# harryjfowen/PointsToWood

Measured on AMD Instinct MI355X. Metric: classified points/sec, higher is better.
Workload: dtype f16x3

## Files before the change

### pointstowood_amd/csrc/p2w_hgemm.h

```cpp
#pragma once
#include "p2w_common.h"
#include <type_traits>

typedef float f32x16 __attribute__((ext_vector_type(16)));
typedef _Float16 h8 __attribute__((ext_vector_type(8)));
typedef __bf16 bf8 __attribute__((ext_vector_type(8)));
typedef __fp16 hpair __attribute__((ext_vector_type(2)));
typedef _Float16 hpairn __attribute__((ext_vector_type(2)));
typedef __bf16 bpair __attribute__((ext_vector_type(2)));
typedef float fpair __attribute__((ext_vector_type(2)));
typedef __attribute__((address_space(3))) void* lds_vp;
typedef const __attribute__((address_space(1))) void* glb_vp;

constexpr int H_BK = 32;
constexpr int SA_EPI_COLS = 1024;

template <int PREC> struct HCfg {
    static constexpr int planes = PREC == 0 ? 2 : 1;
    static constexpr int kslab = PREC == 0 ? 32 : 64;
    static constexpr int kalign = PREC == 0 ? 32 : 64;
};

template <int PREC>
__device__ __forceinline__ f32x16 h_mfma(h8 a, h8 b, f32x16 c) {
    if constexpr (PREC == 2)
        return __builtin_amdgcn_mfma_f32_32x32x16_bf16(__builtin_bit_cast(bf8, a), __builtin_bit_cast(bf8, b), c, 0, 0, 0);
    else
        return __builtin_amdgcn_mfma_f32_32x32x16_f16(a, b, c, 0, 0, 0);
}

typedef float f32x4 __attribute__((ext_vector_type(4)));
template <int PREC>
__device__ __forceinline__ f32x4 h_mfma16(h8 a, h8 b, f32x4 c) {
    if constexpr (PREC == 2)
        return __builtin_amdgcn_mfma_f32_16x16x32_bf16(__builtin_bit_cast(bf8, a), __builtin_bit_cast(bf8, b), c, 0, 0, 0);
    else
        return __builtin_amdgcn_mfma_f32_16x16x32_f16(a, b, c, 0, 0, 0);
}

__device__ __forceinline__ void split_pair(float a, float b, unsigned& hi, unsigned& lo) {
    const hpair h = __builtin_amdgcn_cvt_pkrtz(a, b);
    const fpair rem = {a - (float)h[0], b - (float)h[1]};
    const hpairn l = __builtin_convertvector(rem, hpairn);
    hi = __builtin_bit_cast(unsigned, h);
    lo = __builtin_bit_cast(unsigned, l);
}
template <int PREC>
__device__ __forceinline__ unsigned pack_pair(float a, float b) {
    if constexpr (PREC == 2) {
        const fpair p = {a, b};
        return __builtin_bit_cast(unsigned, __builtin_convertvector(p, bpair));
    } else {
        const fpair p = {__builtin_amdgcn_fmed3f(a, -65504.f, 65504.f), __builtin_amdgcn_fmed3f(b, -65504.f, 65504.f)};
        return __builtin_bit_cast(unsigned, __builtin_convertvector(p, hpairn));
    }
}
template <int PREC>
__device__ __forceinline__ void h_store2(_Float16* __restrict__ base, unsigned ldh, unsigned row, unsigned col, float a, float b) {
    if constexpr (PREC == 0) {
        unsigned hw, lw;
        split_pair(a, b, hw, lw);
        _Float16* p = base + (size_t)row * (2 * ldh) + 64 * (col >> 5) + (col & 31);
        *reinterpret_cast<unsigned*>(p) = hw;
        *reinterpret_cast<unsigned*>(p + 32) = lw;
    } else {
        *reinterpret_cast<unsigned*>(base + (size_t)row * ldh + col) = pack_pair<PREC>(a, b);
    }
}
template <int PREC>
__device__ __forceinline__ void h_store4(_Float16* __restrict__ base, int ldh, size_t row, int col, const float (&v)[4]) {
    if constexpr (PREC == 0) {
        uint2 hi, lo;
        split_pair(v[0], v[1], hi.x, lo.x);
        split_pair(v[2], v[3], hi.y, lo.y);
        _Float16* p = base + row * (size_t)(2 * ldh) + 64 * (col >> 5) + (col & 31);
        *reinterpret_cast<uint2*>(p) = hi;
        *reinterpret_cast<uint2*>(p + 32) = lo;
    } else {
        uint2 w;
        w.x = pack_pair<PREC>(v[0], v[1]);
        w.y = pack_pair<PREC>(v[2], v[3]);
        *reinterpret_cast<uint2*>(base + row * (size_t)ldh + col) = w;
    }
}

__device__ __forceinline__ bool tile_coords_at(int L, int nMt, int nNt, int* mt, int* nt, int mode = 0) {
    const int xcd = L & 7, w = L >> 3;
    if (mode == 0) {
        *mt = xcd + 8 * (w / nNt);
        *nt = w % nNt;
        return *mt < nMt;
    }
    if (nNt >= 8) {
        const int cpx = (nNt + 7) >> 3;
        *mt = w / cpx;
        *nt = xcd + 8 * (w % cpx);
        return *mt < nMt && *nt < nNt;
    }
    const int r = 8 / nNt;
    *nt = xcd % nNt;
    *mt = xcd / nNt + r * w;
    return *mt < nMt;
}
__device__ __forceinline__ bool tile_coords(int nMt, int nNt, int* mt, int* nt, int mode = 0) {
    return tile_coords_at(blockIdx.x, nMt, nNt, mt, nt, mode);
}
static inline int tile_grid(int nMt, int nNt, int mode = 0) {
    if (mode == 0) return 8 * ((nMt + 7) / 8) * nNt;
    if (nNt >= 8) return 8 * nMt * ((nNt + 7) / 8);
    const int r = 8 / nNt;
    return 8 * ((nMt + r - 1) / r);
}
static inline int p2w_cu_count() {
    int dev = 0, n = 256;
    if (hipGetDevice(&dev) == hipSuccess) hipDeviceGetAttribute(&n, hipDeviceAttributeMultiprocessorCount, dev);
    return n > 0 ? n : 256;
}

constexpr int RI_DEPTH = 2;
struct EpiArgs {
    const float *bias, *sc0, *sh0, *sc1, *sh1, *residual;
    int ldr, relu0, relu1, relu2, relu_final;
    const _Float16* res_h;
    unsigned* range;
    const int4* imeta;
};
__device__ __forceinline__ void range_commit(unsigned* __restrict__ dst, bool over, bool seen, int lane) {
    if (lane == 0) {
        unsigned* p = dst + (blockIdx.x & (P2W_RANGE_SLOTS - 1)) * 64;
        if (over) p[0] = 1u;
        if (seen) p[1] = 1u;
    }
}
__device__ __forceinline__ void range_commit_max(unsigned* __restrict__ dst, float m, int lane) {
    range_commit(dst, __ballot(!(m <= P2W_RANGE_HI)) != 0ull, __ballot(m > P2W_RANGE_LO) != 0ull, lane);
}
template <int PREC>
__device__ __forceinline__ fpair h_load2(const _Float16* __restrict__ base, unsigned ldh, unsigned row, unsigned col) {
    if constexpr (PREC == 0) {
        const _Float16* p = base + (size_t)row * (2 * ldh) + 64 * (col >> 5) + (col & 31);
        const hpairn hi = *reinterpret_cast<const hpairn*>(p), lo = *reinterpret_cast<const hpairn*>(p + 32);
        return fpair{(float)hi[0] + (float)lo[0], (float)hi[1] + (float)lo[1]};
    } else if constexpr (PREC == 1) {
        const hpairn v = *reinterpret_cast<const hpairn*>(base + (size_t)row * ldh + col);
        return fpair{(float)v[0], (float)v[1]};
    } else {
        const bpair v = *reinterpret_cast<const bpair*>(base + (size_t)row * ldh + col);
        return fpair{(float)v[0], (float)v[1]};
    }
}
struct OutArgs { float* f32; int ldo; _Float16* h2; int ldh; int hcols; const float* dotw; float* part; int ldpart; };

__device__ __forceinline__ float row16_sum(float v) {
    asm volatile("s_nop 4\n\t"
                 "v_add_f32_dpp %0, %0, %0 quad_perm:[1,0,3,2] row_mask:0xf bank_mask:0xf bound_ctrl:1\n\ts_nop 1\n\t"
                 "v_add_f32_dpp %0, %0, %0 quad_perm:[2,3,0,1] row_mask:0xf bank_mask:0xf bound_ctrl:1\n\ts_nop 1\n\t"
                 "v_add_f32_dpp %0, %0, %0 row_half_mirror row_mask:0xf bank_mask:0xf bound_ctrl:1\n\ts_nop 1\n\t"
                 "v_add_f32_dpp %0, %0, %0 row_mirror row_mask:0xf bank_mask:0xf bound_ctrl:1\n\ts_nop 1"
                 : "+v"(v));
    return v;
}

__device__ __forceinline__ int w_stage_row16(int rho) {
    const int t = rho >> 4, c = rho & 15;
    return 32 * (t >> 1) + 2 * c + (t & 1);
}

template <int PREC, int RT16, int CT16, int EF, bool DOTK = false>
__device__ __forceinline__ void gemm_epilogue_16(const f32x4 (&acc)[RT16][CT16], const EpiArgs& ep, float wscale, int row0, int col0,
                                                 int lane, int M, int N, const OutArgs& o, bool seen_report = true) {
    static_assert(CT16 % 2 == 0, "column tiles come in interleaved pairs");
    constexpr bool GEN = EF < 0;
    constexpr int JQ = CT16 / 2, NSTEP = RT16 * 4;
    const bool R0 = GEN ? ep.relu0 != 0 : (EF & 1) != 0, S0 = GEN ? ep.sc0 != nullptr : (EF & 2) != 0;
    const bool R1 = GEN ? ep.relu1 != 0 : (EF & 4) != 0, S1 = GEN ? ep.sc1 != nullptr : (EF & 8) != 0;
    const bool R2 = GEN ? ep.relu2 != 0 : (EF & 16) != 0;
    const bool RES = !DOTK && (GEN ? (ep.residual != nullptr || ep.res_h != nullptr) : (EF & 32) != 0);
    const bool RF = GEN ? ep.relu_final != 0 : (EF & 64) != 0, OF = GEN ? o.f32 != nullptr : (EF & 128) != 0;
    const bool OH = GEN ? o.h2 != nullptr : (EF & 256) != 0;
    const bool RH = RES && (GEN ? ep.res_h != nullptr : (EF & 1024) != 0);
    constexpr bool RI_OK = !DOTK && RT16 <= 4;
    const bool RI = RI_OK && RES && (GEN ? ep.imeta != nullptr : (EF & 2048) != 0);
// ... 440 lines not shown
    if (out_h2 && (ldh_o & 7)) return P2W_EINVAL;
    const int hcols = ldh_o < (N + KA - 1) / KA * KA ? ldh_o : (N + KA - 1) / KA * KA;
    OutArgs o = {out_f32, ldo, out_h2, ldh_o, hcols, dotw, part, ldpart};
    const int n_cu = p2w_cu_count();
    auto pick_big = [&](int rows) {
        const long tiles256 = (long)p2w_cdiv(rows, 256) * (Npad / 256);
        const long rounds = (tiles256 + n_cu - 1) / n_cu;
        const bool fills = tiles256 * 100 >= rounds * n_cu * 78;
        bool b = N >= 256 && (N % 256) == 0 && tiles256 * 4 >= 3 * n_cu && fills;
        if (flags & P2W_GEMM_TILE_256) b = true;
        if (flags & P2W_GEMM_TILE_128) b = false;
        return b;
    };
    const bool big = pick_big(M);
    bool t64 = false;
    if (!dotw && sk_S == 0 && !ep.imeta && !(flags & (P2W_GEMM_TILE_128 | P2W_GEMM_TILE_256 | P2W_GEMM_NO_TILE_64))) {
        if (flags & P2W_GEMM_TILE_64) t64 = true;
        else if (K <= 1024 && N <= 192) t64 = true;
        else if (K <= 1024 && !big) {
            const long nNt1 = p2w_cdiv(N, 128), T128 = (long)p2w_cdiv(M, 128) * nNt1, T64 = (long)p2w_cdiv(M, 64) * nNt1;
            const long S128 = 2L * n_cu, S64 = 3L * n_cu;
            const double w128 = (double)((T128 + S128 - 1) / S128 * S128) / (double)T128, w64 = (double)((T64 + S64 - 1) / S64 * S64) / (double)T64;
            t64 = T128 <= 2 * S128 && w128 >= 1.3 * w64;
        }
    }
    if (sk_S == 0 && skws && !dotw && !t64 && !(flags & P2W_GEMM_NO_STREAMK)) {
        const int nslab = Kpad / HCfg<PREC>::kslab;
        const double f = PREC == 0 ? 1.0 : 0.7, ts1 = 0.9 * f, ts2 = 1.65 * f, tsb = 2.25 * f;
        auto t_small = [&](long tiles) { return tiles > n_cu ? ts2 : ts1; };
        auto t_big = [&](long tiles) { return tiles >= n_cu ? tsb : (0.75 * f + (tsb - 0.75 * f) * (double)tiles / n_cu); };
        auto one_launch = [&](bool b, int rows) {
            const long T = b ? (long)p2w_cdiv(rows, 256) * (Npad / 256) : (long)p2w_cdiv(rows, 128) * p2w_cdiv(N, 128);
            const long G = b ? n_cu : 2 * n_cu, qq = T / G, R = T % G;
            return (double)nslab * ((double)qq * (b ? tsb : ts2) + (R ? (b ? t_big(R) : t_small(R)) : 0.0));
        };
        const bool big_ok = N >= 256 && (N % 256) == 0;
        double best_cost = one_launch(big, M);
        int best_mode = 0, best_rows_full = 0, best_S = 0;
        bool best_big = big, sk_big = big, tail_big = false;
        double sk_cost = 1e30;
        int sk_rows_full = 0, sk_S_best = 0;
        const size_t piece_b = (size_t)128 * 128 * 4;
        for (int cand = 0; cand < 2; ++cand) {
            const bool b = cand == 0;
            if (b && !(N >= 256 && (N % 256) == 0)) continue;
            if ((flags & P2W_GEMM_TILE_256) && !b) continue;
            if ((flags & P2W_GEMM_TILE_128) && b) continue;
            const int BMm = b ? 256 : 128, G_m = n_cu * (b ? 1 : 2);
            const int nNt_m = b ? Npad / 256 : p2w_cdiv(N, 128), nMt_m = p2w_cdiv(M, BMm);
            const long T = (long)nMt_m * nNt_m, q = T / G_m;
            const int mt_full = (int)((q * G_m) / nNt_m);
            if ((long)mt_full * nNt_m >= T) continue;
            if (q == 0 && b != big) continue;
            const int rows_full = mt_full * BMm, m_t = M - rows_full;
            const double main_t = (double)q * nslab * (b ? tsb : ts2) + (q > 0 ? 4.0 : 0.0);
            const long T_t = (long)p2w_cdiv(m_t, 128) * p2w_cdiv(N, 128);
            if (q > 0) {
                for (int tb = 0; tb < 2; ++tb) {
                    if (tb == 1 && (!big_ok || (flags & P2W_GEMM_TILE_128))) continue;
                    if (tb == 0 && (flags & P2W_GEMM_TILE_256)) continue;
                    const double c = main_t + one_launch(tb == 1, m_t);
                    if (c < 0.95 * best_cost) { best_cost = c; best_mode = 1; best_rows_full = rows_full; best_big = b; best_S = 0; tail_big = tb == 1; }
                }
            }
            for (int S = 2; S <= nslab && T_t * S <= 2 * n_cu; ++S) {
                if ((size_t)(T_t * S) * piece_b > skws_bytes) break;
                const double c = main_t + (double)((nslab + S - 1) / S) * 1.0 * f + 18.0 + (double)(T_t * S) * piece_b * 2.0 / 8.0e6;
                if (c < sk_cost) { sk_cost = c; sk_rows_full = rows_full; sk_big = b; sk_S_best = S; }
            }
        }
        if (sk_S_best > 0 && (sk_cost < 0.9 * best_cost || (flags & P2W_GEMM_STREAMK))) {
            best_mode = 2; best_rows_full = sk_rows_full; best_big = sk_big; best_S = sk_S_best;
        }
        if (best_mode != 0) {
            constexpr int PL = HCfg<PREC>::planes;
            const int fl = (flags & ~(P2W_GEMM_STREAMK | P2W_GEMM_TILE_128 | P2W_GEMM_TILE_256)) | P2W_GEMM_NO_STREAMK;
            const int rows_full = best_rows_full, m_t = M - rows_full;
            if (rows_full > 0) {
                const int32_t rc = launch_gemm_h<PREC>(Ah, ldh_a, Wp, wscale, rows_full, N, K, ep, out_f32, ldo, out_h2, ldh_o,
                                                       fl | (best_big ? P2W_GEMM_TILE_256 : P2W_GEMM_TILE_128), stream);
                if (rc != P2W_OK) return rc;
            }
            const size_t r0 = (size_t)rows_full;
            EpiArgs ept = ep;
            if (ept.imeta) ept.imeta += r0;
            else if (ept.residual) ept.residual += r0 * ep.ldr;
            if (ept.res_h) ept.res_h += r0 * PL * ep.ldr;
            return launch_gemm_h<PREC>(Ah + r0 * PL * ldh_a, ldh_a, Wp, wscale, m_t, N, K, ept, out_f32 ? out_f32 + r0 * ldo : nullptr, ldo,
                                       out_h2 ? out_h2 + r0 * PL * ldh_o : nullptr, ldh_o,
                                       best_mode == 2 ? fl : (fl | (tail_big ? P2W_GEMM_TILE_256 : P2W_GEMM_TILE_128)), stream, nullptr, nullptr, 0,
                                       best_mode == 2 ? skws : nullptr, skws_bytes, best_mode == 2 ? best_S : 0);
        }
    }
    int ef = (ep.relu0 ? 1 : 0) | (ep.sc0 ? 2 : 0) | (ep.relu1 ? 4 : 0) | (ep.sc1 ? 8 : 0) | (ep.relu2 ? 16 : 0) |
             ((ep.residual || ep.res_h) ? 32 : 0) | (ep.relu_final ? 64 : 0) | (out_f32 ? 128 : 0) | (out_h2 ? 256 : 0) | (dotw ? 512 : 0) |
             (ep.res_h ? 1024 : 0) | (ep.imeta ? 2048 : 0);
    const size_t lim = (size_t)1 << 31;
    if ((size_t)M * (size_t)(ldo > 2 * ldh_o ? ldo : 2 * ldh_o) >= lim || ((ep.residual || ep.res_h) && !ep.imeta && (size_t)M * (size_t)ep.ldr * (ep.res_h ? 2 : 1) >= lim) ||
        (N & 1) || (flags & P2W_GEMM_GENERIC_EPI))
        ef = 0;
    auto odd8 = [](const void* q) { return (reinterpret_cast<uintptr_t>(q) & 7) != 0; };
    if ((out_f32 && ((ldo & 1) || odd8(out_f32))) || (ep.residual && ((ep.ldr & 1) || odd8(ep.residual))) || odd8(ep.bias) ||
        (ep.res_h && ((ep.ldr & 7) || (reinterpret_cast<uintptr_t>(ep.res_h) & 15))) ||
        odd8(ep.sc0) || odd8(ep.sh0) || odd8(ep.sc1) || odd8(ep.sh1) || odd8(dotw) || (part && ((ldpart & 3) || (reinterpret_cast<uintptr_t>(part) & 15))))
        ef = 0;
    const size_t w_bytes = (size_t)N * Kpad * 2 * HCfg<PREC>::planes, a_bytes = (size_t)M * Kpad * 2 * HCfg<PREC>::planes;
    auto pick_mode = [&](int nNtx, int nMtx, int per_cu) {
        const bool ok = nNtx >= 8 || (nNtx > 0 && 8 % nNtx == 0);
        if (!ok) return 0;
        if (flags & P2W_GEMM_ORDER_ROWS) return 0;
        if (flags & P2W_GEMM_ORDER_COLS) return 1;
        const size_t l2_keep = (size_t)3 * 1024 * 1024;
        const int wpx = n_cu / 8 * per_cu;
        const int R = wpx / nNtx > 0 ? wpx / nNtx : 1;
        const int rows_px = p2w_cdiv(nMtx, 8), xcds = nMtx < 8 ? nMtx : 8;
        const size_t t_rows = a_bytes * (size_t)p2w_cdiv(nNtx, wpx) + w_bytes * xcds * (w_bytes <= l2_keep ? 1 : p2w_cdiv(rows_px, R));
        size_t t_cols;
        if (nNtx >= 8) {
            const int cpx = p2w_cdiv(nNtx, 8), Rc = wpx / cpx > 0 ? wpx / cpx : 1;
            t_cols = a_bytes * 8 + w_bytes * (w_bytes / 8 <= l2_keep ? 1 : p2w_cdiv(nMtx, Rc));
        } else {
            t_cols = a_bytes * nNtx + w_bytes * 8 / nNtx;
        }
        return t_cols * 10 < t_rows * 9 ? 1 : 0;
    };
    auto pgrid = [&](int nvb, int per_cu) {
        const int cap = n_cu * per_cu;
        int g = nvb < cap ? nvb : cap;
        if (g >= 8) g &= ~7;
        return g;
    };
    if (sk_S > 0) {
        const int nslab = Kpad / HCfg<PREC>::kslab, nNt1 = p2w_cdiv(N, 128), T_t = p2w_cdiv(M, 128) * nNt1;
        gemm_hp_sk_kernel<PREC, 2, 2, 2, 2><<<8 * p2w_cdiv(T_t * sk_S, 8), 256, 0, stream>>>(Ah, ldh_a, Wp, M, Kpad, nNt1, T_t, sk_S, skws);
        gemm_hp_skfix_kernel<PREC, 2, 2, 2, 2><<<T_t * 4, 256, 0, stream>>>(skws, T_t, sk_S, nslab, nNt1, wscale, M, N, ep, o, ef);
    } else if (t64) {
        const int nMt = p2w_cdiv(M, 64), nNt1 = p2w_cdiv(N, 128);
        const int tm = pick_mode(nNt1, nMt, 3), nvb = tile_grid(nMt, nNt1, tm);
        gemm_hp64_kernel<PREC><<<pgrid(nvb, 3), 256, 0, stream>>>(Ah, ldh_a, Wp, wscale, M, N, Kpad, nMt, nNt1, nvb, ep, o, ef, tm);
    } else if (big) {
        const int nMt = p2w_cdiv(M, 256), nNt2 = Npad / 256;
        const int tm = pick_mode(nNt2, nMt, 1), nvb = tile_grid(nMt, nNt2, tm);
        if (dotw) gemm_hp_kernel<PREC, 2, 4, 4, 2, true><<<pgrid(nvb, 1), 512, 0, stream>>>(Ah, ldh_a, Wp, wscale, M, N, Kpad, nMt, nNt2, nvb, ep, o, ef, tm);
        else gemm_hp_kernel<PREC, 2, 4, 4, 2><<<pgrid(nvb, 1), 512, 0, stream>>>(Ah, ldh_a, Wp, wscale, M, N, Kpad, nMt, nNt2, nvb, ep, o, ef, tm);
    } else {
        const int nMt = p2w_cdiv(M, 128), nNt1 = p2w_cdiv(N, 128);
        const int tm = pick_mode(nNt1, nMt, 2), nvb = tile_grid(nMt, nNt1, tm);
        if (dotw) gemm_hp_kernel<PREC, 2, 2, 2, 2, true><<<pgrid(nvb, 2), 256, 0, stream>>>(Ah, ldh_a, Wp, wscale, M, N, Kpad, nMt, nNt1, nvb, ep, o, ef, tm);
        else gemm_hp_kernel<PREC, 2, 2, 2, 2><<<pgrid(nvb, 2), 256, 0, stream>>>(Ah, ldh_a, Wp, wscale, M, N, Kpad, nMt, nNt1, nvb, ep, o, ef, tm);
    }
    return P2W_LAUNCH_STATUS();
}

template <int RT, int GPT> struct SaEpiRegs { float bias[2], s[2], t[2]; int dsc[RT][GPT]; };
template <int PREC, int RT, int G>
__device__ __forceinline__ void sa_epilogue_regs(const f32x16 (&acc)[RT][2], float wscale, int n0, int wc, int lane,
                                                 const SaEpiRegs<RT, 32 / G>& e, int C2, float* __restrict__ out, int ldo,
                                                 _Float16* __restrict__ out_h2, int ldh, float& amax) {
    static_assert(G == 32 || G == 8, "one or four targets per 32-row tile");
    constexpr int GPT = 32 / G;
    const int h = lane >> 5;
#pragma unroll
    for (int i = 0; i < RT; ++i) {
#pragma unroll
        for (int q = 0; q < GPT; ++q) {
            const int dsc = __builtin_amdgcn_readfirstlane(e.dsc[i][q]);
            if (dsc < 0) continue;
            const int tgt = dsc >> 6, d = dsc & 63;
#pragma unroll
            for (int j = 0; j < 2; ++j) {
                const int col = n0 + wc * 64 + j * 32 + (lane & 31);
                const bool cv = col < C2;
                const float sgn = e.s[j] < 0.f ? -1.f : 1.f;
                const fpair sg2 = {sgn, sgn};
                float ext;
                if constexpr (G == 32) {
                    if (d >= 32) {
                        fpair p[8];
#pragma unroll
                        for (int u = 0; u < 8; ++u) p[u] = fpair{acc[i][j][2 * u], acc[i][j][2 * u + 1]} * sg2;
                        float m0 = fmaxf(fmaxf(p[0][0], p[0][1]), p[1][0]);
                        float m1 = fmaxf(fmaxf(p[1][1], p[2][0]), p[2][1]);
                        float m2 = fmaxf(fmaxf(p[3][0], p[3][1]), p[4][0]);
                        float m3 = fmaxf(fmaxf(p[4][1], p[5][0]), p[5][1]);
                        m0 = fmaxf(fmaxf(m0, p[6][0]), p[6][1]);
                        m1 = fmaxf(fmaxf(m1, p[7][0]), p[7][1]);
                        ext = fmaxf(fmaxf(m0, m1), fmaxf(m2, m3));
                    } else {
                        ext = -INFINITY;
#pragma unroll
                        for (int r = 0; r < 16; ++r) {
                            const int slot = (r & 3) + 8 * (r >> 2) + 4 * h;
                            if (slot < d) ext = fmaxf(ext, sgn * acc[i][j][r]);
                        }
                    }
                } else {
                    ext = -INFINITY;
#pragma unroll
                    for (int r = 0; r < 4; ++r) {
                        const int slot = r + 4 * h;
                        if (slot < d) ext = fmaxf(ext, sgn * acc[i][j][4 * q + r]);
                    }
                }
                {
                    const auto sw = __builtin_amdgcn_permlane32_swap(__float_as_uint(ext), __float_as_uint(ext), false, false);
                    ext = fmaxf(__uint_as_float(sw[0]), __uint_as_float(sw[1]));
                }
                float vmax = fmaf(fmaxf(fmaf(sgn * ext, wscale, e.bias[j]), 0.f), e.s[j], e.t[j]);
                if (d == 0 || !cv) vmax = 0.f;
                amax = fmaxf(amax, fabsf(vmax));
                if (cv && h == 0 && out) out[(size_t)tgt * ldo + col] = vmax;
                if (out_h2) {
                    const float nb = __uint_as_float(__builtin_amdgcn_update_dpp(0, __float_as_uint(vmax), 0xB1, 0xf, 0xf, false));
                    if (h == 0 && (lane & 1) == 0 && col < ldh) h_store2<PREC>(out_h2, ldh, tgt, col, vmax, nb);
                }
            }
        }
    }
}

template <int PREC, int BN, int RT, int G>
__global__ __launch_bounds__(512, 2) void sa_conv16p_kernel(const float* __restrict__ P, int ldp, const int* __restrict__ meta_j,
                                                            const float4* __restrict__ meta_g, const int* __restrict__ desc,
                                                            const int* __restrict__ tiles_dev, int M, const float* __restrict__ w1r4, int C1, int C1pad,
                                                            const _Float16* __restrict__ W2h, size_t plane, float wscale, int C2,
                                                            int nMt_, int nNt, const float* __restrict__ b2,
                                                            const float* __restrict__ bn_s, const float* __restrict__ bn_t,
                                                            float* __restrict__ out, int ldo, _Float16* __restrict__ out_h2,
                                                            int ldh, unsigned* __restrict__ range) {
    constexpr int NP = HCfg<PREC>::planes;
    constexpr int WCn = BN / 64, BM = 32 * RT * (8 / WCn), NW = 8, NR = BM / 128;
    constexpr int GPT = 32 / G;
    if (tiles_dev) M = *tiles_dev;
    const int nMt = tiles_dev ? (M + BM / 32 - 1) / (BM / 32) : nMt_;
    if (M <= 0) return;
    constexpr int A_CH = 4 * NP * BM, STAGE_CH = A_CH + 4 * NP * BN;
    constexpr int NWI = 4;
    constexpr int NI = (4 * NP * BN) / 64 / NWI;
    static_assert(NI >= 1, "every issuing wave has at least one W2 DMA piece per slab");
    __shared__ __attribute__((aligned(16))) char S[2 * STAGE_CH * 16 + 4 * 512 * 4 + 3 * SA_EPI_COLS * 4];
    float* const Wr = reinterpret_cast<float*>(S + 2 * STAGE_CH * 16);
    float* const Ep = Wr + 4 * 512;
    const int tid = threadIdx.x, lane = tid & 63;
    for (int i = tid; i < 4 * C1pad; i += 512) Wr[i] = w1r4[i];
    for (int i = tid; i < C2; i += 512) { Ep[i] = b2[i]; Ep[SA_EPI_COLS + i] = bn_s[i]; Ep[2 * SA_EPI_COLS + i] = bn_t[i]; }
    const int wave = __builtin_amdgcn_readfirstlane(tid >> 6), wr = wave / WCn, wc = wave % WCn;
    const int nitems = nMt * nNt, nslab = C1pad / H_BK;
    int first, stride, limit;
    if ((gridDim.x & 7) == 0) {
        const int xcd = blockIdx.x & 7, slot = blockIdx.x >> 3, per = gridDim.x >> 3;
        const int chunk = (nitems + 7) >> 3;
        first = xcd * chunk + slot; stride = per; limit = min((xcd + 1) * chunk, nitems);
    } else {
        first = blockIdx.x; stride = gridDim.x; limit = nitems;
    }
    if (first >= limit) return;
    const int my_items = (limit - first + stride - 1) / stride;
    const int total = my_items * nslab;

    auto item_mt = [&](int it) { return (first + it * stride) / nNt; };
    auto item_nt = [&](int it) { return (first + it * stride) % nNt; };

    constexpr int RCH = 4 * NP;
    auto img = [](int row, int chunk) { return (row * RCH + (NP == 2 ? (chunk ^ ((row >> 1) & 7)) : (chunk ^ ((row >> 2) & 3)))) * 16; };
    auto imgA = [](int row, int chunk) { return (row * RCH + (NP == 2 ? (chunk ^ ((row >> 1) & 7) ^ ((row & 1) << 2)) : (chunk ^ ((row >> 2) & 3)))) * 16; };
    const int prow = tid >> 2, pq = tid & 3;
    const int a_dst = imgA(prow, pq);
    size_t boff[NI];
    int dstc[NI];
    (void)plane;
#pragma unroll
    for (int i = 0; i < NI; ++i) {
        const int g2 = (wave % NWI) + NWI * i;
        const int row = (NP == 2 ? 8 : 16) * g2 + (lane >> (NP == 2 ? 3 : 2));
        const int c = NP == 2 ? ((lane & 7) ^ ((row >> 1) & 7)) : ((lane & 3) ^ ((row >> 2) & 3));
        boff[i] = (size_t)row * (NP * C1pad) + 8 * c;
        dstc[i] = A_CH + g2 * 64;
    }
    constexpr int KADV = NP == 2 ? 2 : 1;
    auto issue = [&](int stage, const _Float16* wbase, int k0) {
        if (wave >= NWI) return;
#pragma unroll
        for (int i = 0; i < NI; ++i)
            __builtin_amdgcn_global_load_lds((glb_vp)(wbase + boff[i] + KADV * k0),
                                             (lds_vp)(S + ((size_t)stage * STAGE_CH + dstc[i]) * 16), 16, 0, 0);
    };
    struct Meta { int j[NR]; float4 g[NR]; };
    struct Vals { float4 v[NR][2]; };
    const int last_row = M * 32 - 1;
    auto load_meta = [&](int mt_, Meta& m) {
#pragma unroll
        for (int u = 0; u < NR; ++u) {
            const int row = min(mt_ * BM + prow + 128 * u, last_row);
            m.j[u] = meta_j[row];
            m.g[u] = meta_g[row];
        }
    };
    auto gather = [&](const Meta& m, int k0, Vals& dst) {
        const unsigned k4 = (unsigned)(k0 >> 2) + 2u * pq;
#pragma unroll
        for (int u = 0; u < NR; ++u) {
            const float4* p = reinterpret_cast<const float4*>(P) + ((unsigned)m.j[u] + k4);
            dst.v[u][0] = p[0];
            dst.v[u][1] = p[1];
        }
    };
    struct WRegs { float4 w[2][4]; };
    auto load_w = [&](int k0, WRegs& wr_) {
        const int k = k0 + 8 * pq;
#pragma unroll
        for (int half = 0; half < 2; ++half)
#pragma unroll
            for (int c = 0; c < 4; ++c) wr_.w[half][c] = *reinterpret_cast<const float4*>(&Wr[c * C1pad + k + 4 * half]);
    };
    const unsigned lds_base = (unsigned)(uintptr_t)(lds_vp)S;
    auto produce = [&](int stage, const Meta& m, int k0, const Vals& src, const WRegs& wr_) {
        const int k = k0 + 8 * pq;
#pragma unroll
      for (int u = 0; u < NR; ++u) {
        const float4 rg = m.g[u];
        unsigned hiw[4], low[4];
#pragma unroll
        for (int half = 0; half < 2; ++half) {
            const int kk = k + 4 * half;
            const float4 wx = wr_.w[half][0], wy = wr_.w[half][1], wz = wr_.w[half][2], wf = wr_.w[half][3];
            const float4 p = src.v[u][half];
            const float gx = rg.x, gy = rg.y, gz = rg.z, gw = rg.w;
            float v[4];
            v[0] = fmaxf(fmaf(gw, wf.x, fmaf(gz, wz.x, fmaf(gy, wy.x, fmaf(gx, wx.x, p.x)))), 0.f);
            v[1] = fmaxf(fmaf(gw, wf.y, fmaf(gz, wz.y, fmaf(gy, wy.y, fmaf(gx, wx.y, p.y)))), 0.f);
            v[2] = fmaxf(fmaf(gw, wf.z, fmaf(gz, wz.z, fmaf(gy, wy.z, fmaf(gx, wx.z, p.z)))), 0.f);
            v[3] = fmaxf(fmaf(gw, wf.w, fmaf(gz, wz.w, fmaf(gy, wy.w, fmaf(gx, wx.w, p.w)))), 0.f);
            if constexpr (PREC == 0) {
                unsigned h01, l01, h23, l23;
                split_pair(v[0], v[1], h01, l01);
                split_pair(v[2], v[3], h23, l23);
                hiw[2 * half] = h01; hiw[2 * half + 1] = h23;
                low[2 * half] = l01; low[2 * half + 1] = l23;
            } else {
                hiw[2 * half] = pack_pair<PREC>(v[0], v[1]); hiw[2 * half + 1] = pack_pair<PREC>(v[2], v[3]);
            }
        }
        const unsigned sa = lds_base + (unsigned)stage * (STAGE_CH * 16) + (unsigned)(a_dst + u * 128 * RCH * 16);
        {
            typedef unsigned u32x4 __attribute__((ext_vector_type(4)));
            const u32x4 hv = {hiw[0], hiw[1], hiw[2], hiw[3]};
            asm volatile("ds_write_b128 %0, %1" :: "v"(sa), "v"(hv) : "memory");
            if constexpr (PREC == 0) {
                const u32x4 lv = {low[0], low[1], low[2], low[3]};
                asm volatile("ds_write_b128 %0, %1" :: "v"(sa ^ 64u), "v"(lv) : "memory");
            }
        }
      }
    };

    const int r = lane & 31, h = lane >> 5;
    int offA[RT], offB[2];
#pragma unroll
    for (int t = 0; t < RT; ++t) offA[t] = imgA(wr * 32 * RT + 32 * t + r, h);
#pragma unroll
    for (int t = 0; t < 2; ++t) offB[t] = A_CH * 16 + img(wc * 64 + 32 * t + r, h);
    f32x16 acc[RT][2];
#pragma unroll
    for (int i = 0; i < RT; ++i)
#pragma unroll
        for (int j = 0; j < 2; ++j)
#pragma unroll
            for (int e = 0; e < 16; ++e) acc[i][j][e] = 0.f;

    struct Cur { int it, s, mt, nt; };
    auto nxt = [&](Cur c) {
        if (++c.s == nslab) {
            c.s = 0; ++c.it;
            const int itc = min(c.it, my_items - 1);
            c.mt = item_mt(itc); c.nt = item_nt(itc);
        }
        return c;
    };
    auto meta_of = [&](Cur c, Meta& m) { load_meta(c.mt, m); };
    auto k_of = [&](Cur c) { return (c.it < my_items ? c.s : nslab - 1) * H_BK; };
    Cur c0 = {0, 0, item_mt(0), item_nt(0)}, c1 = nxt(c0), c2 = nxt(c1), c3 = nxt(c2);
    Meta ma, mb, mc;
    Vals va;
    {
        Meta m0;
        meta_of(c0, m0);
        meta_of(c1, ma);
        meta_of(c2, mb);
        meta_of(c3, mc);
        __syncthreads();
        issue(0, W2h + (size_t)c0.nt * BN * NP * C1pad, 0);
        gather(m0, 0, va);
        WRegs w0;
        load_w(0, w0);
        produce(0, m0, 0, va, w0);
        gather(ma, k_of(c1), va);
#pragma unroll
        for (int u = 0; u < NR; ++u)
#pragma unroll
            for (int hh = 0; hh < 2; ++hh)
                asm volatile("" : "+v"(va.v[u][hh].x), "+v"(va.v[u][hh].y), "+v"(va.v[u][hh].z), "+v"(va.v[u][hh].w));
    }
    struct Degs { int d[RT][GPT]; };
    auto load_deg = [&](int mt_, Degs& e) {
#pragma unroll
        for (int i = 0; i < RT; ++i)
#pragma unroll
            for (int q = 0; q < GPT; ++q) e.d[i][q] = desc[min(mt_ * (BM / 32) + wr * RT + i, M - 1) * GPT + q];
    };
    Degs dg_;
    load_deg(c0.mt, dg_);
    float amax = 0.f;
    for (int g = 0; g < total; ++g) {
        asm volatile("" ::: "memory");
        __builtin_amdgcn_s_waitcnt(0xC07F);
        __builtin_amdgcn_s_barrier();
        asm volatile("" ::: "memory");
        Vals vb;
        gather(mb, k_of(c2), vb);
        meta_of(c3, mc);
        Degs dg_n;
        load_deg(c1.mt, dg_n);
        WRegs wk;
        load_w(k_of(c1), wk);
        __builtin_amdgcn_sched_barrier(0);
        if (g + 1 < total)
            issue((g + 1) & 1, W2h + (size_t)c1.nt * BN * NP * C1pad, c1.s * H_BK);
        const char* st = S + (size_t)(g & 1) * STAGE_CH * 16;
        h8 afq[2][NP][RT], bfq[2][NP][2];
#pragma unroll
        for (int kk = 0; kk < 2; ++kk)
#pragma unroll
            for (int p = 0; p < NP; ++p) {
#pragma unroll
                for (int t = 0; t < RT; ++t) afq[kk][p][t] = *reinterpret_cast<const h8*>(st + (offA[t] ^ (kk << 5) ^ (p << 6)));
#pragma unroll
                for (int t = 0; t < 2; ++t) bfq[kk][p][t] = *reinterpret_cast<const h8*>(st + (offB[t] ^ (kk << 5) ^ (p << 6)));
            }
#pragma unroll
        for (int kk = 0; kk < 2; ++kk) {
            auto& af = afq[kk];
            auto& bf = bfq[kk];
#pragma unroll
            for (int i = 0; i < RT; ++i)
#pragma unroll
                for (int j = 0; j < 2; ++j) {
                    if constexpr (PREC == 0) {
                        acc[i][j] = h_mfma<PREC>(af[1][i], bf[0][j], acc[i][j]);
                        acc[i][j] = h_mfma<PREC>(af[0][i], bf[1][j], acc[i][j]);
                    }
                    acc[i][j] = h_mfma<PREC>(af[0][i], bf[0][j], acc[i][j]);
                }
            if (kk == 0) {
                produce((g + 1) & 1, ma, k_of(c1), va, wk);
                constexpr int NM = 2 * RT * (PREC == 0 ? 3 : 1);
#pragma unroll
                for (int q = 0; q < NM; ++q) {
                    __builtin_amdgcn_sched_group_barrier(0x008, 1, 0);
                    __builtin_amdgcn_sched_group_barrier(0x002, (PREC == 0 ? 16 : 40) * NR / RT, 0);
                }
                __builtin_amdgcn_sched_barrier(0);
            }
        }
#pragma unroll
        for (int u = 0; u < NR; ++u) {
            asm volatile("" : "+v"(vb.v[u][0].x), "+v"(vb.v[u][0].y), "+v"(vb.v[u][0].z), "+v"(vb.v[u][0].w),
                              "+v"(vb.v[u][1].x), "+v"(vb.v[u][1].y), "+v"(vb.v[u][1].z), "+v"(vb.v[u][1].w));
            asm volatile("" : "+v"(mc.j[u]), "+v"(mc.g[u].x), "+v"(mc.g[u].y), "+v"(mc.g[u].z), "+v"(mc.g[u].w));
        }
#pragma unroll
        for (int i = 0; i < RT; ++i)
#pragma unroll
            for (int q = 0; q < GPT; ++q) asm volatile("" : "+v"(dg_n.d[i][q]));
        __builtin_amdgcn_s_waitcnt(p2w_vmcnt_imm(0));
        if (c0.s == nslab - 1) {
            SaEpiRegs<RT, GPT> e;
#pragma unroll
            for (int j = 0; j < 2; ++j) {
                const int col = min(c0.nt * BN + wc * 64 + j * 32 + (lane & 31), C2 - 1);
                e.bias[j] = Ep[col]; e.s[j] = Ep[SA_EPI_COLS + col]; e.t[j] = Ep[2 * SA_EPI_COLS + col];
            }
#pragma unroll
            for (int i = 0; i < RT; ++i)
#pragma unroll
                for (int q = 0; q < GPT; ++q) e.dsc[i][q] = (c0.mt * (BM / 32) + wr * RT + i >= M) ? -1 : dg_.d[i][q];
            sa_epilogue_regs<PREC, RT, G>(acc, wscale, c0.nt * BN, wc, lane, e, C2, out, ldo, out_h2, ldh, amax);
#pragma unroll
            for (int i = 0; i < RT; ++i)
#pragma unroll
                for (int j = 0; j < 2; ++j)
#pragma unroll
                    for (int e2 = 0; e2 < 16; ++e2) acc[i][j][e2] = 0.f;
        }
        __builtin_amdgcn_sched_barrier(0);
        va = vb; ma = mb; mb = mc; dg_ = dg_n;
        c0 = c1; c1 = c2; c2 = c3; c3 = nxt(c3);
    }
    if (range) range_commit_max(range, amax, lane);
}


__global__ __launch_bounds__(256) void sa_edge_meta_kernel(const float4* __restrict__ xyzr, const int* __restrict__ idx, const int* __restrict__ batch_dst,
                                    const float* __restrict__ sf, const int* __restrict__ nbr, const int* __restrict__ deg, int kw,
                                    int M, int n_src, int ldp4, int G, const int* __restrict__ list, const int* __restrict__ n_list_dev,
                                    const int* __restrict__ src_row, int* __restrict__ meta_j, float4* __restrict__ meta_g, int* __restrict__ desc,
                                    float4* __restrict__ zero_row);
constexpr int SA_PART_BLOCK = 1024;
__global__ __launch_bounds__(SA_PART_BLOCK) void sa_part_count_kernel(const int* __restrict__ deg, int kw, int M, int* __restrict__ blk_small);
__global__ __launch_bounds__(1024) void sa_part_scan_kernel(int* __restrict__ blk_small, int nblk, int M, int* __restrict__ counts);
__global__ __launch_bounds__(SA_PART_BLOCK) void sa_part_scatter_kernel(const int* __restrict__ deg, int kw, int M, const int* __restrict__ blk_small,
                                                                     int* __restrict__ list_small, int* __restrict__ list_large);

static inline size_t sa_conv_ws_bytes(long M, int flags) {
    const long tiles32 = M, tiles8 = (M + 3) / 4;
    if (!(flags & P2W_SA_PACK8)) return (size_t)(tiles32 * 32 * 20 + tiles32 * 4 + 256);
    const long nblk = (M + SA_PART_BLOCK - 1) / SA_PART_BLOCK;
    return (size_t)((tiles32 + tiles8) * 32 * 20 + (tiles32 + tiles8 * 4) * 4 + 2 * M * 4 + nblk * 4 + 64 + 1024);
}

template <int PREC>
static int32_t launch_sa_conv_h(const float* P, int32_t ldp, int32_t n_src, const float* xyzr_src, const int32_t* idx, const int32_t* batch_dst,
                                const float* sf, const int32_t* nbr, const int32_t* deg, int32_t kw, int32_t M,
                                const float* w1r4, const _Float16* W2h, float wscale, int32_t C1, int32_t C2, const float* b2,
                                const float* bn_s, const float* bn_t, float* out, int32_t ldo, _Float16* out_h2, int32_t ldh,
                                void* ws, size_t ws_bytes, int32_t flags, hipStream_t stream, const int32_t* src_row = nullptr,
                                unsigned* range = nullptr) {
    constexpr int KA = HCfg<PREC>::kalign;
    const int C2pad = (C2 + 255) / 256 * 256, C1pad = (C1 + KA - 1) / KA * KA;
    if (C1pad > 512 || C2 > SA_EPI_COLS || (long)M >= (1L << 25) || ((long)n_src + 1) * (ldp / 4) >= (1L << 31)) return P2W_EUNSUPPORTED;
    if (ldp < C1pad) return P2W_EINVAL;
    if (ws == nullptr || ws_bytes < sa_conv_ws_bytes(M, flags)) return P2W_EWORKSPACE;
    if (reinterpret_cast<uintptr_t>(ws) & 15u) return P2W_EALIGN;
    const int n_cu = p2w_cu_count();
    const bool wide = (flags & (P2W_SA_ITEM_256 | P2W_SA_ITEM_128)) ? (flags & P2W_SA_ITEM_256) != 0 : C2 > 128;
    const int tpi = wide ? 4 : 8, nNt3 = p2w_cdiv(C2, wide ? 256 : 128);
    const float4* x4 = reinterpret_cast<const float4*>(xyzr_src);
    auto run = [&](auto g_c, const int* list, const int* n_list_dev, const int* tiles_dev, long tiles_max, float4* meta_g, int* meta_j,
                   int* desc) {
        constexpr int G = decltype(g_c)::value;
        const long rows_max = tiles_max * 32;
        sa_edge_meta_kernel<<<p2w_cdiv(rows_max, 256), 256, 0, stream>>>(x4, idx, batch_dst, sf, nbr, deg, kw, M, n_src, ldp / 4, G,
                                                                       list, n_list_dev, src_row, meta_j, meta_g, desc,
                                                                       reinterpret_cast<float4*>(const_cast<float*>(P) + (size_t)n_src * ldp));
        const long items = p2w_cdiv(tiles_max, tpi) * nNt3;
        int grid = (int)(items < n_cu ? items : n_cu);
        if (grid >= 8) grid &= ~7;
        const int nMt3 = (int)p2w_cdiv(tiles_max, tpi);
        if (wide)
            sa_conv16p_kernel<PREC, 256, 2, G><<<grid, 512, 0, stream>>>(
                P, ldp, meta_j, meta_g, desc, tiles_dev, (int)tiles_max, w1r4, C1, C1pad, W2h, (size_t)C2pad * C1pad, wscale, C2, nMt3,
                nNt3, b2, bn_s, bn_t, out, ldo, out_h2, ldh, range);
        else
            sa_conv16p_kernel<PREC, 128, 2, G><<<grid, 512, 0, stream>>>(
                P, ldp, meta_j, meta_g, desc, tiles_dev, (int)tiles_max, w1r4, C1, C1pad, W2h, (size_t)C2pad * C1pad, wscale, C2, nMt3,
                nNt3, b2, bn_s, bn_t, out, ldo, out_h2, ldh, range);
    };
    char* w = static_cast<char*>(ws);
    if (!(flags & P2W_SA_PACK8)) {
        float4* meta_g = reinterpret_cast<float4*>(w);
        int* meta_j = reinterpret_cast<int*>(meta_g + (size_t)M * 32);
        int* desc = meta_j + (size_t)M * 32;
        run(std::integral_constant<int, 32>{}, nullptr, nullptr, nullptr, M, meta_g, meta_j, desc);
        return P2W_LAUNCH_STATUS();
    }
    const long t32 = M, t8 = (M + 3) / 4, nblk = p2w_cdiv(M, SA_PART_BLOCK);
    float4* mg_l = reinterpret_cast<float4*>(w);            w += t32 * 32 * 16;
    float4* mg_s = reinterpret_cast<float4*>(w);            w += t8 * 32 * 16;
    int* mj_l = reinterpret_cast<int*>(w);                  w += t32 * 32 * 4;
    int* mj_s = reinterpret_cast<int*>(w);                  w += t8 * 32 * 4;
    int* desc_l = reinterpret_cast<int*>(w);                w += t32 * 4;
    int* desc_s = reinterpret_cast<int*>(w);                w += t8 * 4 * 4;
    int* list_s = reinterpret_cast<int*>(w);                w += (size_t)M * 4;
    int* list_l = reinterpret_cast<int*>(w);                w += (size_t)M * 4;
    int* blk = reinterpret_cast<int*>(w);                   w += nblk * 4;
    int* counts = reinterpret_cast<int*>(w);
    sa_part_count_kernel<<<(int)nblk, SA_PART_BLOCK, 0, stream>>>(deg, kw, M, blk);
    sa_part_scan_kernel<<<1, 1024, 0, stream>>>(blk, (int)nblk, M, counts);
    sa_part_scatter_kernel<<<(int)nblk, SA_PART_BLOCK, 0, stream>>>(deg, kw, M, blk, list_s, list_l);
    run(std::integral_constant<int, 8>{}, list_s, counts + 0, counts + 2, t8, mg_s, mj_s, desc_s);
    run(std::integral_constant<int, 32>{}, list_l, counts + 1, counts + 3, t32, mg_l, mj_l, desc_l);
    return P2W_LAUNCH_STATUS();
}

int32_t p2w_gemm_h1_impl(int32_t prec, const _Float16* Ah, int32_t ldh_a, const _Float16* Wp, float wscale, int32_t M, int32_t N,
                         int32_t K, const EpiArgs& ep, float* out_f32, int32_t ldo, _Float16* out_h2, int32_t ldh_o,
                         int32_t flags, hipStream_t stream, const float* dotw = nullptr, float* part = nullptr, int32_t ldpart = 0,
                         float* skws = nullptr, size_t skws_bytes = 0);
int32_t p2w_sa_conv_h1_impl(int32_t prec, const float* P, int32_t ldp, int32_t n_src, const float* xyzr_src, const int32_t* idx,
                            const int32_t* batch_dst, const float* sf, const int32_t* nbr, const int32_t* deg, int32_t kw,
                            int32_t M, const float* w1r4, const _Float16* W2h, float wscale, int32_t C1, int32_t C2,
                            const float* b2, const float* bn_s, const float* bn_t, float* out, int32_t ldo, _Float16* out_h2,
                            int32_t ldh, void* ws, size_t ws_bytes, int32_t flags, hipStream_t stream, const int32_t* src_row = nullptr,
                            unsigned* range = nullptr);
```

Baseline: 20.53 million.

## Switch SA conv kernel from 32x32x16 to 16x16x32 MFMA tiles

Recasts the sa_conv16p kernel's MMA inner loop to use 16x16x32 MFMA instructions on 16-row/16-column subtiles instead of 32x32x16, with new LDS fragment offsets and a single k-step per slab instead of two. The epilogue max-reduction is rewritten for the new accumulator layout, using permlane16 and permlane32 swaps and precomputed per-column signs. It also splits the A-fragment loads into two halves interleaved with MFMA groups and retunes the scheduling hints. The aim is better MFMA throughput and latency hiding, at the cost of more accumulator registers, more fragment loads and a more intricate epilogue.

```diff
diff --git a/pointstowood_amd/csrc/p2w_hgemm.h b/pointstowood_amd/csrc/p2w_hgemm.h
--- a/pointstowood_amd/csrc/p2w_hgemm.h
+++ b/pointstowood_amd/csrc/p2w_hgemm.h
@@ -20,14 +20,6 @@
     static constexpr int kslab = PREC == 0 ? 32 : 64;
     static constexpr int kalign = PREC == 0 ? 32 : 64;
 };
-
-template <int PREC>
-__device__ __forceinline__ f32x16 h_mfma(h8 a, h8 b, f32x16 c) {
-    if constexpr (PREC == 2)
-        return __builtin_amdgcn_mfma_f32_32x32x16_bf16(__builtin_bit_cast(bf8, a), __builtin_bit_cast(bf8, b), c, 0, 0, 0);
-    else
-        return __builtin_amdgcn_mfma_f32_32x32x16_f16(a, b, c, 0, 0, 0);
-}
 
 typedef float f32x4 __attribute__((ext_vector_type(4)));
 template <int PREC>
@@ -774,67 +766,86 @@
     return P2W_LAUNCH_STATUS();
 }
 
-template <int RT, int GPT> struct SaEpiRegs { float bias[2], s[2], t[2]; int dsc[RT][GPT]; };
+template <int RT, int GPT> struct SaEpiRegs { float sgn[4], bias[GPT == 1 ? 1 : 2], s[GPT == 1 ? 1 : 2], t[GPT == 1 ? 1 : 2]; int dsc[RT][GPT]; };
 template <int PREC, int RT, int G>
-__device__ __forceinline__ void sa_epilogue_regs(const f32x16 (&acc)[RT][2], float wscale, int n0, int wc, int lane,
+__device__ __forceinline__ void sa_epilogue_regs(const f32x4 (&acc)[2 * RT][4], float wscale, int n0, int wc, int lane,
                                                  const SaEpiRegs<RT, 32 / G>& e, int C2, float* __restrict__ out, int ldo,
                                                  _Float16* __restrict__ out_h2, int ldh, float& amax) {
     static_assert(G == 32 || G == 8, "one or four targets per 32-row tile");
-    constexpr int GPT = 32 / G;
-    const int h = lane >> 5;
+    constexpr int NU = G == 32 ? 1 : 2;
+    constexpr int NC = G == 32 ? 1 : 2;
+    const int kg = lane >> 4;
 #pragma unroll
     for (int i = 0; i < RT; ++i) {
 #pragma unroll
-        for (int q = 0; q < GPT; ++q) {
-            const int dsc = __builtin_amdgcn_readfirstlane(e.dsc[i][q]);
-            if (dsc < 0) continue;
-            const int tgt = dsc >> 6, d = dsc & 63;
-#pragma unroll
-            for (int j = 0; j < 2; ++j) {
-                const int col = n0 + wc * 64 + j * 32 + (lane & 31);
-                const bool cv = col < C2;
-                const float sgn = e.s[j] < 0.f ? -1.f : 1.f;
-                const fpair sg2 = {sgn, sgn};
+        for (int u = 0; u < NU; ++u) {
+            int dsc;
+            if constexpr (G == 32) {
+                dsc = __builtin_amdgcn_readfirstlane(e.dsc[i][0]);
+                if (dsc < 0) continue;
+            } else {
+                const int d0 = __builtin_amdgcn_readfirstlane(e.dsc[i][2 * u]), d1 = __builtin_amdgcn_readfirstlane(e.dsc[i][2 * u + 1]);
+                if (d0 < 0 && d1 < 0) continue;
+                dsc = (kg >> 1) ? d1 : d0;
+            }
+            const bool tv = dsc >= 0;
+            const int tgt = dsc >> 6, d = tv ? (dsc & 63) : 0;
+            auto in_lane = [&](int j) {
+                const float sgn = e.sgn[j];
                 float ext;
                 if constexpr (G == 32) {
+                    const f32x4 &a0 = acc[2 * i][j], &a1 = acc[2 * i + 1][j];
                     if (d >= 32) {
-                        fpair p[8];
-#pragma unroll
-                        for (int u = 0; u < 8; ++u) p[u] = fpair{acc[i][j][2 * u], acc[i][j][2 * u + 1]} * sg2;
-                        float m0 = fmaxf(fmaxf(p[0][0], p[0][1]), p[1][0]);
-                        float m1 = fmaxf(fmaxf(p[1][1], p[2][0]), p[2][1]);
-                        float m2 = fmaxf(fmaxf(p[3][0], p[3][1]), p[4][0]);
-                        float m3 = fmaxf(fmaxf(p[4][1], p[5][0]), p[5][1]);
-                        m0 = fmaxf(fmaxf(m0, p[6][0]), p[6][1]);
-                        m1 = fmaxf(fmaxf(m1, p[7][0]), p[7][1]);
-                        ext = fmaxf(fmaxf(m0, m1), fmaxf(m2, m3));
+                        const fpair sg2 = {sgn, sgn};
+                        const fpair p0 = fpair{a0[0], a0[1]} * sg2, p1 = fpair{a0[2], a0[3]} * sg2;
+                        const fpair p2 = fpair{a1[0], a1[1]} * sg2, p3 = fpair{a1[2], a1[3]} * sg2;
+                        float m0 = fmaxf(fmaxf(p0[0], p0[1]), p1[0]);
+                        float m1 = fmaxf(fmaxf(p1[1], p2[0]), p2[1]);
+                        m0 = fmaxf(fmaxf(m0, p3[0]), p3[1]);
+                        ext = fmaxf(m0, m1);
                     } else {
                         ext = -INFINITY;
 #pragma unroll
-                        for (int r = 0; r < 16; ++r) {
-                            const int slot = (r & 3) + 8 * (r >> 2) + 4 * h;
-                            if (slot < d) ext = fmaxf(ext, sgn * acc[i][j][r]);
+                        for (int r = 0; r < 4; ++r) {
+                            const int slot = 4 * kg + r;
+                            if (slot < d) ext = fmaxf(ext, sgn * a0[r]);
+                            if (slot + 16 < d) ext = fmaxf(ext, sgn * a1[r]);
                         }
                     }
                 } else {
+                    const f32x4& a = acc[2 * i + u][j];
                     ext = -INFINITY;
 #pragma unroll
                     for (int r = 0; r < 4; ++r) {
-                        const int slot = r + 4 * h;
-                        if (slot < d) ext = fmaxf(ext, sgn * acc[i][j][4 * q + r]);
+                        const int slot = 4 * (kg & 1) + r;
+                        if (slot < d) ext = fmaxf(ext, sgn * a[r]);
                     }
                 }
-                {
-                    const auto sw = __builtin_amdgcn_permlane32_swap(__float_as_uint(ext), __float_as_uint(ext), false, false);
-                    ext = fmaxf(__uint_as_float(sw[0]), __uint_as_float(sw[1]));
-                }
-                float vmax = fmaf(fmaxf(fmaf(sgn * ext, wscale, e.bias[j]), 0.f), e.s[j], e.t[j]);
+                return ext;
+            };
+            auto pair16 = [](float a, float b) {
+                const auto sw = __builtin_amdgcn_permlane16_swap(__float_as_uint(a), __float_as_uint(b), false, false);
+                return fmaxf(__uint_as_float(sw[0]), __uint_as_float(sw[1]));
+            };
+            float x = pair16(in_lane(0), in_lane(1));
+            const float y = pair16(in_lane(2), in_lane(3));
+            if constexpr (G == 32) {
+                const auto sw = __builtin_amdgcn_permlane32_swap(__float_as_uint(x), __float_as_uint(y), false, false);
+                x = fmaxf(__uint_as_float(sw[0]), __uint_as_float(sw[1]));
+            }
+#pragma unroll
+            for (int c = 0; c < NC; ++c) {
+                const int col = n0 + wc * 64 + (G == 32 ? lane : 32 * c + (lane & 31));
+                const bool cv = col < C2;
+                const float sgn = e.s[c] < 0.f ? -1.f : 1.f;
+                const float ext = c == 0 ? x : y;
+                float vmax = fmaf(fmaxf(fmaf(sgn * ext, wscale, e.bias[c]), 0.f), e.s[c], e.t[c]);
                 if (d == 0 || !cv) vmax = 0.f;
                 amax = fmaxf(amax, fabsf(vmax));
-                if (cv && h == 0 && out) out[(size_t)tgt * ldo + col] = vmax;
+                if (tv && cv && out) out[(size_t)tgt * ldo + col] = vmax;
                 if (out_h2) {
                     const float nb = __uint_as_float(__builtin_amdgcn_update_dpp(0, __float_as_uint(vmax), 0xB1, 0xf, 0xf, false));
-                    if (h == 0 && (lane & 1) == 0 && col < ldh) h_store2<PREC>(out_h2, ldh, tgt, col, vmax, nb);
+                    if (tv && (lane & 1) == 0 && col < ldh) h_store2<PREC>(out_h2, ldh, tgt, col, vmax, nb);
                 }
             }
         }
@@ -976,19 +987,18 @@
       }
     };
 
-    const int r = lane & 31, h = lane >> 5;
-    int offA[RT], offB[2];
-#pragma unroll
-    for (int t = 0; t < RT; ++t) offA[t] = imgA(wr * 32 * RT + 32 * t + r, h);
-#pragma unroll
-    for (int t = 0; t < 2; ++t) offB[t] = A_CH * 16 + img(wc * 64 + 32 * t + r, h);
-    f32x16 acc[RT][2];
-#pragma unroll
-    for (int i = 0; i < RT; ++i)
-#pragma unroll
-        for (int j = 0; j < 2; ++j)
-#pragma unroll
-            for (int e = 0; e < 16; ++e) acc[i][j][e] = 0.f;
+    constexpr int RT16 = 2 * RT, CT16 = 4;
+    const int r16 = lane & 15, kg = lane >> 4;
+    int offA[RT16], offB[CT16];
+#pragma unroll
+    for (int t = 0; t < RT16; ++t) offA[t] = imgA(wr * 32 * RT + 16 * t + r16, kg);
+#pragma unroll
+    for (int t = 0; t < CT16; ++t) offB[t] = A_CH * 16 + img(wc * 64 + 16 * t + r16, kg);
+    f32x4 acc[RT16][CT16];
+#pragma unroll
+    for (int i = 0; i < RT16; ++i)
+#pragma unroll
+        for (int j = 0; j < CT16; ++j) acc[i][j] = f32x4{0.f, 0.f, 0.f, 0.f};
 
     struct Cur { int it, s, mt, nt; };
     auto nxt = [&](Cur c) {
@@ -1049,37 +1059,35 @@
         if (g + 1 < total)
             issue((g + 1) & 1, W2h + (size_t)c1.nt * BN * NP * C1pad, c1.s * H_BK);
         const char* st = S + (size_t)(g & 1) * STAGE_CH * 16;
-        h8 afq[2][NP][RT], bfq[2][NP][2];
-#pragma unroll
-        for (int kk = 0; kk < 2; ++kk)
-#pragma unroll
-            for (int p = 0; p < NP; ++p) {
-#pragma unroll
-                for (int t = 0; t < RT; ++t) afq[kk][p][t] = *reinterpret_cast<const h8*>(st + (offA[t] ^ (kk << 5) ^ (p << 6)));
-#pragma unroll
-                for (int t = 0; t < 2; ++t) bfq[kk][p][t] = *reinterpret_cast<const h8*>(st + (offB[t] ^ (kk << 5) ^ (p << 6)));
-            }
-#pragma unroll
-        for (int kk = 0; kk < 2; ++kk) {
-            auto& af = afq[kk];
-            auto& bf = bfq[kk];
-#pragma unroll
-            for (int i = 0; i < RT; ++i)
-#pragma unroll
-                for (int j = 0; j < 2; ++j) {
-                    if constexpr (PREC == 0) {
-                        acc[i][j] = h_mfma<PREC>(af[1][i], bf[0][j], acc[i][j]);
-                        acc[i][j] = h_mfma<PREC>(af[0][i], bf[1][j], acc[i][j]);
-                    }
-                    acc[i][j] = h_mfma<PREC>(af[0][i], bf[0][j], acc[i][j]);
-                }
-            if (kk == 0) {
+        h8 af[NP][RT16], bf[NP][CT16];
+        constexpr int HR = RT16 / 2;
+#pragma unroll
+        for (int p = 0; p < NP; ++p) {
+#pragma unroll
+            for (int t = 0; t < CT16; ++t) bf[p][t] = *reinterpret_cast<const h8*>(st + (offB[t] ^ (p << 6)));
+#pragma unroll
+            for (int t = 0; t < HR; ++t) af[p][t] = *reinterpret_cast<const h8*>(st + (offA[t] ^ (p << 6)));
+        }
+#pragma unroll
+        for (int p = 0; p < NP; ++p)
+#pragma unroll
+            for (int t = HR; t < RT16; ++t) af[p][t] = *reinterpret_cast<const h8*>(st + (offA[t] ^ (p << 6)));
+#pragma unroll
+        for (int hh = 0; hh < 2; ++hh) {
+#pragma unroll
+            for (int term = (PREC == 0 ? 0 : 2); term < 3; ++term)
+#pragma unroll
+                for (int i = hh * HR; i < (hh + 1) * HR; ++i)
+#pragma unroll
+                    for (int j = 0; j < CT16; ++j)
+                        acc[i][j] = h_mfma16<PREC>(af[term == 0 ? NP - 1 : 0][i], bf[term == 1 ? NP - 1 : 0][j], acc[i][j]);
+            if (hh == 0) {
                 produce((g + 1) & 1, ma, k_of(c1), va, wk);
-                constexpr int NM = 2 * RT * (PREC == 0 ? 3 : 1);
+                constexpr int NM = HR * CT16 * (PREC == 0 ? 3 : 1);
 #pragma unroll
                 for (int q = 0; q < NM; ++q) {
                     __builtin_amdgcn_sched_group_barrier(0x008, 1, 0);
-                    __builtin_amdgcn_sched_group_barrier(0x002, (PREC == 0 ? 16 : 40) * NR / RT, 0);
+                    __builtin_amdgcn_sched_group_barrier(0x002, (PREC == 0 ? 8 : 20) * NR / RT, 0);
                 }
                 __builtin_amdgcn_sched_barrier(0);
             }
@@ -1098,9 +1106,12 @@
         if (c0.s == nslab - 1) {
             SaEpiRegs<RT, GPT> e;
 #pragma unroll
-            for (int j = 0; j < 2; ++j) {
-                const int col = min(c0.nt * BN + wc * 64 + j * 32 + (lane & 31), C2 - 1);
-                e.bias[j] = Ep[col]; e.s[j] = Ep[SA_EPI_COLS + col]; e.t[j] = Ep[2 * SA_EPI_COLS + col];
+            for (int j = 0; j < 4; ++j)
+                e.sgn[j] = Ep[SA_EPI_COLS + min(c0.nt * BN + wc * 64 + j * 16 + (lane & 15), C2 - 1)] < 0.f ? -1.f : 1.f;
+#pragma unroll
+            for (int c = 0; c < (GPT == 1 ? 1 : 2); ++c) {
+                const int col = min(c0.nt * BN + wc * 64 + (GPT == 1 ? lane : 32 * c + (lane & 31)), C2 - 1);
+                e.bias[c] = Ep[col]; e.s[c] = Ep[SA_EPI_COLS + col]; e.t[c] = Ep[2 * SA_EPI_COLS + col];
             }
 #pragma unroll
             for (int i = 0; i < RT; ++i)
@@ -1108,11 +1119,9 @@
                 for (int q = 0; q < GPT; ++q) e.dsc[i][q] = (c0.mt * (BM / 32) + wr * RT + i >= M) ? -1 : dg_.d[i][q];
             sa_epilogue_regs<PREC, RT, G>(acc, wscale, c0.nt * BN, wc, lane, e, C2, out, ldo, out_h2, ldh, amax);
 #pragma unroll
-            for (int i = 0; i < RT; ++i)
-#pragma unroll
-                for (int j = 0; j < 2; ++j)
-#pragma unroll
-                    for (int e2 = 0; e2 < 16; ++e2) acc[i][j][e2] = 0.f;
+            for (int i = 0; i < RT16; ++i)
+#pragma unroll
+                for (int j = 0; j < CT16; ++j) acc[i][j] = f32x4{0.f, 0.f, 0.f, 0.f};
         }
         __builtin_amdgcn_sched_barrier(0);
         va = vb; ma = mb; mb = mc; dg_ = dg_n;
```

Result: no change. 20.58 million, median of 2 (+0.2%).
